# SamsungLabs/nb-asr

Measured on AMD Instinct MI355X. Metric: utterances_per_sec, higher is better.
Workload: dtype f32

## Files before the change

### nb_asr_amd/csrc/gemm_conv_split.hip

```cpp
#include "storage.h"

#include <cstdlib>

#include <type_traits>

namespace nbasr {

typedef float floatx4 __attribute__((ext_vector_type(4)));

constexpr int PB_CI = 16, PB_TAPS = 8;
constexpr int pb_frames(int nj) { return 64 * nj; }
constexpr int pb_rows(int mi) { return 32 * mi; }
constexpr int PB_THREADS = 512;

struct SplitBf16x3 {
    static constexpr int NS = 3;
    typedef __bf16 vec8 __attribute__((ext_vector_type(8)));
    static constexpr bool SCALED = false;
    __host__ __device__ static constexpr int taps_per_step(int stride) { return stride == 1 ? 4 : 2; }
    __device__ static __forceinline__ void split(float v, unsigned short (&s)[NS]) {
        const __bf16 hi = static_cast<__bf16>(v);
        const float r1 = v - static_cast<float>(hi);
        const __bf16 mid = static_cast<__bf16>(r1);
        const __bf16 lo = static_cast<__bf16>(r1 - static_cast<float>(mid));
        s[0] = __builtin_bit_cast(unsigned short, hi);
        s[1] = __builtin_bit_cast(unsigned short, mid);
        s[2] = __builtin_bit_cast(unsigned short, lo);
    }
    __device__ static __forceinline__ floatx4 mfma(vec8 a, vec8 b, floatx4 c) {
        return __builtin_amdgcn_mfma_f32_16x16x32_bf16(a, b, c, 0, 0, 0);
    }
    static constexpr const char* NAME = "nbasr_dense_conv1d_packed(bf16x3)";
};

struct SplitF16x2 {
    static constexpr int NS = 2;
    typedef _Float16 vec8 __attribute__((ext_vector_type(8)));
    static constexpr bool SCALED = true;
    __host__ __device__ static constexpr int taps_per_step(int) { return 4; }
    __device__ static __forceinline__ void split(float v, unsigned short (&s)[NS]) {
        const _Float16 hi = static_cast<_Float16>(v);
        const _Float16 lo = static_cast<_Float16>(v - static_cast<float>(hi));
        s[0] = __builtin_bit_cast(unsigned short, hi);
        s[1] = __builtin_bit_cast(unsigned short, lo);
    }
    __device__ static __forceinline__ floatx4 mfma(vec8 a, vec8 b, floatx4 c) {
        return __builtin_amdgcn_mfma_f32_16x16x32_f16(a, b, c, 0, 0, 0);
    }
    static constexpr const char* NAME = "nbasr_dense_conv1d_packed(f16x2)";
};

struct PlainBf16 {
    static constexpr int NS = 1;
    typedef __bf16 vec8 __attribute__((ext_vector_type(8)));
    static constexpr bool SCALED = false;
    __host__ __device__ static constexpr int taps_per_step(int) { return 8; }
    __device__ static __forceinline__ void split(float v, unsigned short (&s)[NS]) {
        s[0] = __builtin_bit_cast(unsigned short, static_cast<__bf16>(v));
    }
    __device__ static __forceinline__ floatx4 mfma(vec8 a, vec8 b, floatx4 c) {
        return __builtin_amdgcn_mfma_f32_16x16x32_bf16(a, b, c, 0, 0, 0);
    }
    static constexpr const char* NAME = "nbasr_dense_conv1d_packed(bf16)";
};

template <class P> constexpr bool has_image_path() { return P::SCALED || P::NS == 1; }

template <class P> constexpr size_t pb_group_bytes(int mi) { return static_cast<size_t>(P::NS) * PB_TAPS * pb_rows(mi) * PB_CI * 2; }

template <class P, int S, int MI = 4, int NJ = 4>
struct GeoP {
    static constexpr int PBM = pb_rows(MI);
    static constexpr int PBN = pb_frames(NJ);
    static constexpr int TP = P::taps_per_step(S);
    static constexpr int QSTEPS = PB_TAPS / TP;
    static constexpr int A_STEP_BYTES = P::NS * TP * PBM * PB_CI * 2;
    static constexpr int XR = (PBN - 1) * S + PB_TAPS;
    static constexpr int XRH = (XR + 1) / 2;
    static constexpr int ROWS = (S == 1) ? XR : 2 * XRH;
    static constexpr int RP = (ROWS + 15) / 16 * 16;
    static constexpr int X_BYTES = P::NS * RP * PB_CI * 2;
    static constexpr int NQUADS = ((XR + 3 + 3) / 4 + 7) / 8 * 8;
    static constexpr int XITEMS = NQUADS * (PB_CI / 2);
    static constexpr int NCHUNK = QSTEPS > 1 ? QSTEPS - 1 : 1;
    static constexpr int XI = (XITEMS + PB_THREADS * NCHUNK - 1) / (PB_THREADS * NCHUNK);
    static constexpr int RING = 2;
    static constexpr int OPERAND_BYTES = RING * (A_STEP_BYTES + X_BYTES);
    static constexpr int STAGING_BYTES = 8 * 32 * 68 * 4;
    static constexpr int LDS_BYTES = OPERAND_BYTES > STAGING_BYTES ? OPERAND_BYTES : STAGING_BYTES;
    __device__ static constexpr int rowmap(int row) { return (S == 1) ? row : (row & 1) * XRH + (row >> 1); }
};

struct PackedConvArgs {
    const float* x; const unsigned char* wp; const float* bias;
    const float* s0; const float* s1; const float* s2;
    float* y;
    int c_in, frames_in, ld_in, c_out, frames_out, ld_out, lpad;
    int n_groups, n_mt, n_nt, batch;
    LnRef ln_x;
    const float* x_absmax;
    const float* w_inv_scale;
    int x_is_image;
    const float* x_range;
    int sel_want;
    int staged_epilogue;
    float* part;
};

__device__ __forceinline__ bool range_is_extreme(const float* r) { return r[2] != 0.f || r[1] < r[0] * 2.44140625e-04f; }

__host__ __device__ inline void pow2_normaliser(float absmax, int target, float& scale, float& inv)
{
    unsigned bits;
    __builtin_memcpy(&bits, &absmax, 4);
    const int e = static_cast<int>((bits >> 23) & 0xffu);
    int k = (bits & 0x7fffffffu) ? (127 + target) - e : 0;
    k = k > 126 ? 126 : (k < -126 ? -126 : k);
    const unsigned sb = static_cast<unsigned>(127 + k) << 23, ib = static_cast<unsigned>(127 - k) << 23;
    __builtin_memcpy(&scale, &sb, 4);
    __builtin_memcpy(&inv, &ib, 4);
}

__device__ __forceinline__ unsigned pack2(unsigned short a, unsigned short b) {
    return static_cast<unsigned>(a) | (static_cast<unsigned>(b) << 16);
}

__global__ __launch_bounds__(256) void weight_row_scales_kernel(const float* __restrict__ w, float* __restrict__ scales,
                                                                int c_out, int row_elems, int rows)
{
    __shared__ float s_max[4];
    const int co = blockIdx.x;
    float m = 0.f;
    if (co < c_out)
        for (int i = threadIdx.x; i < row_elems; i += 256) m = fmaxf(m, fabsf(w[static_cast<size_t>(co) * row_elems + i]));
#pragma unroll
    for (int d = 32; d >= 1; d >>= 1) m = fmaxf(m, __shfl_xor(m, d));
    if ((threadIdx.x & 63) == 0) s_max[threadIdx.x >> 6] = m;
    __syncthreads();
    if (threadIdx.x == 0) {
        float scale, inv;
        pow2_normaliser(fmaxf(fmaxf(s_max[0], s_max[1]), fmaxf(s_max[2], s_max[3])), 13, scale, inv);
        scales[co] = scale;
        scales[rows + co] = inv;
    }
}

template <class P>
__global__ __launch_bounds__(256) void pack_dense_weights_kernel(const float* __restrict__ w, unsigned short* __restrict__ wp,
                                                                 const float* __restrict__ row_scale,
                                                                 int c_out, int c_in, int n_mt, int n_groups, int PB_TP, int PB_M)
{
    const int PB_QSTEPS = PB_TAPS / PB_TP;
    const long long total = static_cast<long long>(n_mt) * n_groups * PB_QSTEPS * PB_TP * PB_M * PB_CI;
    for (long long i = static_cast<long long>(blockIdx.x) * blockDim.x + threadIdx.x; i < total;
         i += static_cast<long long>(gridDim.x) * blockDim.x) {
        long long e = i;
        const int ci_l = e % PB_CI; e /= PB_CI;
        const int co_l = e % PB_M; e /= PB_M;
        const int tp = e % PB_TP; e /= PB_TP;
        const int q = e % PB_QSTEPS; e /= PB_QSTEPS;
        const int g = e % n_groups; e /= n_groups;
        const int mt = static_cast<int>(e);
        const int co = mt * PB_M + co_l, ci = g * PB_CI + ci_l, tap = q * PB_TP + tp;
        float v = (co < c_out && ci < c_in) ? w[(static_cast<size_t>(co) * c_in + ci) * PB_TAPS + tap] : 0.f;
        if (P::SCALED) v *= row_scale[co];
        unsigned short s[P::NS];
        P::split(v, s);
        const size_t step = (static_cast<size_t>(mt) * n_groups + g) * PB_QSTEPS + q;
#pragma unroll
        for (int k = 0; k < P::NS; ++k)
            wp[((((step * P::NS + k) * PB_TP + tp) * 2 + (ci_l >> 3)) * PB_M + co_l) * 8 + (ci_l & 7)] = s[k];
    }
}

template <class P, int S, bool LNX, bool XIMG = false, int MI = 4, int NJ = 4>
__global__ __launch_bounds__(PB_THREADS, 2) void gemm_conv_split_kernel(const PackedConvArgs a)
{
    static_assert(NJ == 4 || (NJ == 2 && XIMG && P::NS == 2) || (NJ == 8 && XIMG && P::NS == 1),
                  "128-frame tiles exist for the fp16 image path only, 512-frame tiles for the one-term bf16 flavour only");
    static_assert(!(XIMG && LNX) && !(XIMG && !has_image_path<P>()), "the image path: scaled fp16 scheme or plain bf16, no LayerNorm on load");
    static_assert(XIMG || P::NS > 1, "plain bf16 operands exist as an image only");
    static_assert(MI == 4 || ((MI == 5 || MI == 3 || MI == 2) && XIMG), "160-, 96- and 64-row tiles exist for the image path only");
    using G = GeoP<P, S, MI, NJ>;
    constexpr int PB_M = G::PBM, WROWS = 16 * MI;
    constexpr int PB_N = G::PBN, WCOLS = 16 * NJ;
    using vec8 = typename P::vec8;
    constexpr int TP = G::TP, QS = G::QSTEPS, ASTEP = G::A_STEP_BYTES;
    extern __shared__ __attribute__((aligned(16))) unsigned char smem[];
    unsigned char* const Abuf = smem;
    unsigned char* const Xbase = smem + G::RING * ASTEP;

    const int nwg = gridDim.x, id = blockIdx.x;
    const int xq = nwg >> 3, xr = nwg & 7, xcd = id & 7;
    const int L = (xcd < xr ? xcd * (xq + 1) : xr * (xq + 1) + (xcd - xr) * xq) + (id >> 3);
    int mt_i, b, nt_i;
    {
        mt_i = L % a.n_mt;
        const int rest = L / a.n_mt;
        b = rest / a.n_nt;
        nt_i = rest - b * a.n_nt;
    }
    const int m0 = mt_i * PB_M, n0 = nt_i * PB_N;
    if (a.x_range && a.sel_want >= 0 && static_cast<int>(range_is_extreme(a.x_range + 4 * b)) != a.sel_want) return;

    const int tid = threadIdx.x;
    const int lane = tid & 63;
    const int wave = __builtin_amdgcn_readfirstlane(tid >> 6);
    const int wm = wave >> 2, wn = wave & 3;
    const bool older = wave < 4;

    const float* __restrict__ xb = a.x + static_cast<size_t>(b) * a.c_in * a.ld_in;
    const int tin0 = n0 * S - a.lpad;
    const float* __restrict__ xstats = LNX ? a.ln_x.stats + static_cast<size_t>(b) * 2 * a.ld_in : nullptr;
    const unsigned char* __restrict__ wtile = a.wp + static_cast<size_t>(mt_i) * a.n_groups * pb_group_bytes<P>(MI);

    const bool wave_active = (m0 + wm * WROWS) < a.c_out && (n0 + wn * WCOLS) < a.ld_out;

    floatx4 acc[MI][NJ], tot[MI][NJ];
#pragma unroll
    for (int i = 0; i < MI; ++i)
#pragma unroll
        for (int j = 0; j < NJ; ++j)
#pragma unroll
            for (int r = 0; r < 4; ++r) { acc[i][j][r] = 0.f; tot[i][j][r] = 0.f; }
    auto flush_group = [&]() {
        if constexpr (P::NS > 1) {
#pragma unroll
            for (int i = 0; i < MI; ++i)
#pragma unroll
                for (int j = 0; j < NJ; ++j)
#pragma unroll
                    for (int r = 0; r < 4; ++r) { tot[i][j][r] += acc[i][j][r]; acc[i][j][r] = 0.f; }
        }
    };

    auto dma_weights = [&](int step, int buf) {
        const unsigned char* src = wtile + static_cast<size_t>(step) * ASTEP;
#pragma unroll
        for (int j = 0; j < ASTEP / 1024 / 8; ++j) {
            const int chunk = wave * (ASTEP / 1024 / 8) + j;
            __builtin_amdgcn_global_load_lds(
                (const __attribute__((address_space(1))) void*)(src + chunk * 1024 + lane * 16),
                (__attribute__((address_space(3))) void*)(Abuf + buf * ASTEP + chunk * 1024),
                16, 0, 0);
        }
    };
    auto dma_x = [&](int g, int xbuf, int q) {
        constexpr int NP = (G::X_BYTES + 1023) / 1024;
        const unsigned char* img = reinterpret_cast<const unsigned char*>(a.x) +
                                   (static_cast<size_t>(b) * a.n_groups + g) * (2 * P::NS) * static_cast<size_t>(a.ld_in + 1) * 16;
#pragma unroll 1
        for (int i = wave * QS + q; i < NP; i += 8 * QS) {
            const int o = i * 1024 + lane * 16;
            if (o < G::X_BYTES) {
                const int plane = o / (G::RP * 16), rr = (o - plane * (G::RP * 16)) >> 4;
                const int frame = tin0 + (S == 1 ? rr : 2 * (rr % G::XRH) + rr / G::XRH);
                const int row = (rr < G::ROWS && frame >= 0 && frame < a.ld_in) ? frame + 1 : 0;
                __builtin_amdgcn_global_load_lds(
                    (const __attribute__((address_space(1))) void*)(img + (static_cast<size_t>(plane) * (a.ld_in + 1) + row) * 16),
                    (__attribute__((address_space(3))) void*)(Xbase + xbuf * G::X_BYTES + i * 1024), 16, 0, 0);
            }
        }
    };
    floatx4 xreg[G::XI][2];
    const int a0 = tin0 & ~3, xoff = tin0 - a0;
    float x_scale = 1.f, x_inv = 1.f;
    if constexpr (P::SCALED) pow2_normaliser(a.x_range ? a.x_range[4 * b] : a.x_absmax[b], 14, x_scale, x_inv);
    auto load_x = [&](int g, int c) {
#pragma unroll
        for (int i = 0; i < G::XI; ++i) {
            const int e = tid + PB_THREADS * (c * G::XI + i);
            const int p = (e >> 3) & 7;
            const int t = a0 + 4 * ((e >> 6) * 8 + (e & 7));
            const int ci = g * PB_CI + 2 * p;
            const bool ok = e < G::XITEMS && t >= 0 && t < a.ld_in;
            floatx4 v0 = {0.f, 0.f, 0.f, 0.f}, v1 = {0.f, 0.f, 0.f, 0.f};
            if (ok && ci < a.c_in) v0 = *reinterpret_cast<const floatx4*>(xb + static_cast<size_t>(ci) * a.ld_in + t);
            if (ok && ci + 1 < a.c_in) v1 = *reinterpret_cast<const floatx4*>(xb + static_cast<size_t>(ci + 1) * a.ld_in + t);
            if (LNX && ok) {
                const floatx4 mean = *reinterpret_cast<const floatx4*>(xstats + t);
                const floatx4 rstd = *reinterpret_cast<const floatx4*>(xstats + a.ld_in + t);
                if (ci < a.c_in) {
                    const float gm = a.ln_x.gamma[ci], bt = a.ln_x.beta[ci];
#pragma unroll
                    for (int j = 0; j < 4; ++j) v0[j] = ln_apply(v0[j], mean[j], rstd[j], gm, bt);
                }
                if (ci + 1 < a.c_in) {
                    const float gm = a.ln_x.gamma[ci + 1], bt = a.ln_x.beta[ci + 1];
#pragma unroll
                    for (int j = 0; j < 4; ++j) v1[j] = ln_apply(v1[j], mean[j], rstd[j], gm, bt);
                }
            }
            if constexpr (P::SCALED) { v0 *= x_scale; v1 *= x_scale; }
            xreg[i][0] = v0;
            xreg[i][1] = v1;
        }
    };
    auto commit_x = [&](int xbuf, int c) {
        unsigned* const X = reinterpret_cast<unsigned*>(Xbase + xbuf * G::X_BYTES);
#pragma unroll
        for (int i = 0; i < G::XI; ++i) {
            const int e = tid + PB_THREADS * (c * G::XI + i);
            const int p = (e >> 3) & 7;
            const int row0 = 4 * ((e >> 6) * 8 + (e & 7)) - xoff;
            if (e >= G::XITEMS) continue;
            unsigned* const col = X + (p >> 2) * G::RP * 4 + (p & 3);
#pragma unroll
            for (int j = 0; j < 4; ++j) {
                const int row = row0 + j;
                if (row < 0 || row >= G::XR) continue;
                unsigned short s0[P::NS], s1[P::NS];
                P::split(xreg[i][0][j], s0);
                P::split(xreg[i][1][j], s1);
                unsigned* dst = col + G::rowmap(row) * 4;
#pragma unroll
                for (int k = 0; k < P::NS; ++k) dst[k * 2 * G::RP * 4] = pack2(s0[k], s1[k]);
            }
        }
    };

    const int l15 = lane & 15, kq = lane >> 4;
    const int a_lane = (((kq >> 1) * 2 + (kq & 1)) * PB_M + wm * WROWS + l15) * 16;
    const int x_lane = (kq & 1) * G::RP * 16;

    constexpr bool PIPE = P::NS <= 2;
    auto mma_step = [&](int q, int abuf, int xbuf) {
        const unsigned char* A = Abuf + abuf * ASTEP + a_lane;
        const unsigned char* X = Xbase + xbuf * G::X_BYTES + x_lane;
        auto read_b = [&](int pp, int j, vec8 (&f)[P::NS]) {
            const int row = G::rowmap((wn * WCOLS + j * 16 + l15) * S + q * TP + 2 * pp + (kq >> 1));
#pragma unroll
            for (int k = 0; k < P::NS; ++k) f[k] = *reinterpret_cast<const vec8*>(X + (k * 2 * G::RP + row) * 16);
        };
        auto read_a = [&](int pp, int i, vec8 (&f)[P::NS]) {
#pragma unroll
            for (int k = 0; k < P::NS; ++k) f[k] = *reinterpret_cast<const vec8*>(A + ((k * TP + 2 * pp) * 2 * PB_M + i * 16) * 16);
        };
        auto block = [&](int i, int j, const vec8 (&af)[P::NS], const vec8 (&bf)[P::NS]) {
            floatx4 c = acc[i][j];
            if constexpr (P::NS == 3) {
                c = P::mfma(af[2], bf[0], c);
                c = P::mfma(af[0], bf[2], c);
                c = P::mfma(af[1], bf[1], c);
            }
            if constexpr (P::NS > 1) {
                c = P::mfma(af[1], bf[0], c);
                c = P::mfma(af[0], bf[1], c);
            }
            acc[i][j] = P::mfma(af[0], bf[0], c);
        };
        if constexpr (PIPE) {
            vec8 bfr[NJ][P::NS], af[2][P::NS];
#pragma unroll
            for (int j = 0; j < NJ; ++j) read_b(0, j, bfr[j]);
            read_a(0, 0, af[0]);
#pragma unroll
            for (int pp = 0; pp < TP / 2; ++pp) {
#pragma unroll
                for (int i = 0; i < MI; ++i) {
                    const int cur = (pp * MI + i) & 1;
                    const bool more_a = i < MI - 1 || pp + 1 < TP / 2;
#pragma unroll
                    for (int j = 0; j < NJ; ++j) {
                        __builtin_amdgcn_sched_barrier(0);
                        block(i, j, af[cur], bfr[j]);
                        __builtin_amdgcn_sched_barrier(0);
                        if (j == 0 && more_a) read_a(i < MI - 1 ? pp : pp + 1, (i + 1) % MI, af[cur ^ 1]);
                        if (i == MI - 1 && pp + 1 < TP / 2) read_b(pp + 1, j, bfr[j]);
                    }
                }
            }
            __builtin_amdgcn_sched_barrier(0);
        } else {
#pragma unroll 1
            for (int pp = 0; pp < TP / 2; ++pp) {
                vec8 bfr[NJ][P::NS];
#pragma unroll
                for (int j = 0; j < NJ; ++j) read_b(pp, j, bfr[j]);
#pragma unroll
                for (int i = 0; i < MI; ++i) {
                    vec8 af[P::NS];
                    read_a(pp, i, af);
#pragma unroll
                    for (int j = 0; j < NJ; ++j) block(i, j, af, bfr[j]);
                }
            }
        }
    };

    const int ng = a.n_groups;
    dma_weights(0, 0);
    if constexpr (XIMG) {
#pragma unroll 1
        for (int q = 0; q < QS; ++q) dma_x(0, 0, q);
    } else {
#pragma unroll 1
        for (int c = 0; c < G::NCHUNK; ++c) { load_x(0, c); commit_x(0, c); }
    }
    asm volatile("s_waitcnt vmcnt(0)" ::: "memory");
    __syncthreads();

    if (!older) __builtin_amdgcn_s_setprio(1);
    int step = 0;
    for (int g = 0; g < ng; ++g) {
        const bool more = g + 1 < ng;
#pragma unroll 1
        for (int q = 0; q < QS; ++q, ++step) {
            const bool prefetch = q + 1 < QS || more;
            const bool chunk = more && q < QS - 1;
            if (older) {
                if constexpr (XIMG) {
                    if (more) dma_x(g + 1, (g + 1) & 1, q);
                } else {
                    if (more && q >= 1) commit_x((g + 1) & 1, q - 1);
                    if (chunk) load_x(g + 1, q);
                }
                if (prefetch) dma_weights(step + 1, (step + 1) & 1);
            } else if (!XIMG && chunk) {
                load_x(g + 1, q);
            }
            if (wave_active) mma_step(q, step & 1, g & 1);
            if (!older) {
                if constexpr (XIMG) {
                    if (more) dma_x(g + 1, (g + 1) & 1, q);
                } else {
                    if (chunk) commit_x((g + 1) & 1, q);
                }
                if (prefetch) dma_weights(step + 1, (step + 1) & 1);
            }
            asm volatile("s_waitcnt vmcnt(0)" ::: "memory");
            __syncthreads();
        }
        flush_group();
    }

    if constexpr (P::NS == 1) {
        constexpr int TSH = WCOLS + 8;
        constexpr int LPR = WCOLS / 8, RPI = 64 / LPR;
        unsigned short* const T = reinterpret_cast<unsigned short*>(smem) + wave * (32 * TSH);
        static_assert(8 * 32 * TSH * 2 <= G::LDS_BYTES, "output staging must fit the operand buffers");
        if (wave_active) {
            bf16_t* const yb = reinterpret_cast<bf16_t*>(a.y);
            const int n = n0 + wn * WCOLS + (lane % LPR) * 8;
#pragma unroll
            for (int i0 = 0; i0 < MI; i0 += 2) {
#pragma unroll
                for (int ii = 0; ii < 2; ++ii) {
                    const int i = i0 + ii;
                    if (i >= MI) break;
#pragma unroll
                    for (int j = 0; j < NJ; ++j) {
                        const bool live = n0 + wn * WCOLS + j * 16 + l15 < a.frames_out;
#pragma unroll
                        for (int r = 0; r < 4; ++r) {
                            const int m = m0 + wm * WROWS + i * 16 + kq * 4 + r;
                            const float v = (live && m < a.c_out) ? relu_clamp(acc[i][j][r] + a.bias[m]) : 0.f;
                            T[(ii * 16 + kq * 4 + r) * TSH + j * 16 + l15] = __builtin_bit_cast(unsigned short, static_cast<__bf16>(v));
                        }
                    }
                }
                asm volatile("s_waitcnt lgkmcnt(0)" ::: "memory");
                const int rows_pass = (MI - i0 >= 2) ? 32 : 16;
#pragma unroll
                for (int it = 0; it < 32 / RPI; ++it) {
                    const int ml = it * RPI + lane / LPR, m = m0 + wm * WROWS + i0 * 16 + ml;
                    if (ml < rows_pass && m < a.c_out && n < a.ld_out) {
                        const u4v t = *reinterpret_cast<const u4v*>(T + ml * TSH + (lane % LPR) * 8);
                        *reinterpret_cast<u4v*>(yb + (static_cast<size_t>(b) * a.c_out + m) * a.ld_out + n) = t;
                    }
                }
                asm volatile("s_waitcnt lgkmcnt(0)" ::: "memory");
            }
        }
        return;
    } else {
    if (!a.s0 && !a.s1 && !a.s2 && a.staged_epilogue) {
        constexpr int TS = WCOLS + 4;
        constexpr int FQ = WCOLS / 4, RI = 64 / FQ, NIT = 32 / RI;
        float* const T = reinterpret_cast<float*>(smem) + wave * (32 * TS);
        static_assert(8 * 32 * TS * 4 <= G::LDS_BYTES, "output staging must fit the operand buffers");
        if (!wave_active) return;
        const int nc = n0 + wn * WCOLS + (lane % FQ) * 4;
        const bool want_stats = a.part != nullptr;
        const int scol = lane % WCOLS, usel = lane / WCOLS;
        const int ncol = n0 + wn * WCOLS + scol;
#pragma unroll
        for (int i0 = 0; i0 < MI; i0 += 2) {
#pragma unroll
            for (int ii = 0; ii < 2; ++ii) {
                const int i = i0 + ii;
                if (i >= MI) break;
#pragma unroll
                for (int j = 0; j < NJ; ++j) {
                    const bool live = n0 + wn * WCOLS + j * 16 + l15 < a.frames_out;
#pragma unroll
                    for (int r = 0; r < 4; ++r) {
                        const int m = m0 + wm * WROWS + i * 16 + kq * 4 + r;
                        float v = 0.f;
                        if (live && m < a.c_out) {
                            float sum = tot[i][j][r];
                            if constexpr (P::SCALED) sum = sum * x_inv * a.w_inv_scale[m];
                            v = relu_clamp(sum + a.bias[m]);
                        }
                        T[(ii * 16 + kq * 4 + r) * TS + j * 16 + l15] = v;
                    }
                }
            }
            asm volatile("s_waitcnt lgkmcnt(0)" ::: "memory");
            const int rows_pass = (MI - i0 >= 2) ? 32 : 16;
#pragma unroll
            for (int it = 0; it < NIT; ++it) {
                const int ml = it * RI + lane / FQ;
                const int m = m0 + wm * WROWS + i0 * 16 + ml;
                if (ml < rows_pass && m < a.c_out && nc < a.ld_out) {
                    const floatx4 t = *reinterpret_cast<const floatx4*>(T + ml * TS + (lane % FQ) * 4);
                    *reinterpret_cast<floatx4*>(a.y + (static_cast<size_t>(b) * a.c_out + m) * a.ld_out + nc) = t;
                }
            }
            if (want_stats) {
#pragma unroll
                for (int u0 = 0; u0 < 2; u0 += 64 / WCOLS) {
                    const int u = u0 + usel;
                    const int mu = m0 + wm * WROWS + (i0 + u) * 16;
                    if (i0 + u < MI && mu < a.c_out) {
                        const int nrows = min(16, a.c_out - mu);
                        const float c = T[(u * 16) * TS + scol];
                        float s1 = 0.f, s2 = 0.f;
#pragma unroll
                        for (int r = 1; r < 16; ++r) {
                            const float d = (r < nrows) ? T[(u * 16 + r) * TS + scol] - c : 0.f;
                            s1 += d;
                            s2 = __builtin_fmaf(d, d, s2);
                        }
                        if (ncol < a.ld_out) {
                            const float inv = 1.0f / static_cast<float>(nrows);
                            float* prow = a.part + (static_cast<size_t>(mu >> 4) * a.batch + b) * 2 * a.ld_out + ncol;
                            prow[0] = c + s1 * inv;
                            prow[a.ld_out] = s2 - s1 * s1 * inv;
                        }
                    }
                }
            }
            asm volatile("s_waitcnt lgkmcnt(0)" ::: "memory");
        }
        return;
    }
    if (!wave_active) return;
#pragma unroll
    for (int i = 0; i < MI; ++i) {
#pragma unroll
        for (int j = 0; j < NJ; ++j) {
            const int n = n0 + wn * WCOLS + j * 16 + l15;
            if (n >= a.ld_out) continue;
            const bool live = n < a.frames_out;
#pragma unroll
            for (int r = 0; r < 4; ++r) {
                const int m = m0 + wm * WROWS + i * 16 + kq * 4 + r;
                if (m >= a.c_out) continue;
                float sum = tot[i][j][r];
                if constexpr (P::SCALED) sum = sum * x_inv * a.w_inv_scale[m];
                float v = relu_clamp(sum + a.bias[m]);
                const size_t off = (static_cast<size_t>(b) * a.c_out + m) * a.ld_out + n;
                if (a.s0) v += a.s0[off];
                if (a.s1) v += a.s1[off];
                if (a.s2) v += a.s2[off];
                a.y[off] = live ? v : 0.f;
            }
        }
    }
    }
}


template <class P, int S>
static int launch_packed(PackedConvArgs a, hipStream_t stream)
{
    using G = GeoP<P, S>;
    constexpr int PB_M = G::PBM;
    constexpr bool HAS_LNX = !P::SCALED;
    static const hipError_t attr0 = hipFuncSetAttribute(reinterpret_cast<const void*>(gemm_conv_split_kernel<P, S, false>),
                                                        hipFuncAttributeMaxDynamicSharedMemorySize, G::LDS_BYTES);
    static const hipError_t attr1 = hipFuncSetAttribute(reinterpret_cast<const void*>(gemm_conv_split_kernel<P, S, HAS_LNX>),
                                                        hipFuncAttributeMaxDynamicSharedMemorySize, G::LDS_BYTES);
    const hipError_t attr = attr0 != hipSuccess ? attr0 : attr1;
    if (attr != hipSuccess) {
        set_error("%s: cannot reserve %d bytes of LDS: %s", P::NAME, G::LDS_BYTES, hipGetErrorString(attr));
        return static_cast<int>(attr);
    }
    NBASR_REQUIRE(HAS_LNX || !a.ln_x.stats, NBASR_EINVAL, "%s: this scheme takes no deferred LayerNorm", P::NAME);
    a.n_mt = (a.c_out + PB_M - 1) / PB_M;
    a.n_nt = (a.ld_out + G::PBN - 1) / G::PBN;
    const long long nwg = static_cast<long long>(a.n_mt) * a.n_nt * a.batch;
    NBASR_REQUIRE(nwg < (1ll << 31), NBASR_EINVAL, "%s: too many tiles (%lld)", P::NAME, nwg);
    if (a.ln_x.stats)
        hipLaunchKernelGGL((gemm_conv_split_kernel<P, S, HAS_LNX>), dim3(static_cast<unsigned>(nwg)), dim3(PB_THREADS), G::LDS_BYTES, stream, a);
    else
        hipLaunchKernelGGL((gemm_conv_split_kernel<P, S, false>), dim3(static_cast<unsigned>(nwg)), dim3(PB_THREADS), G::LDS_BYTES, stream, a);
    return launch_status(P::NAME);
}

static inline int rows_to_mi(int row_tile) { return row_tile == 128 ? 4 : (row_tile == 160 ? 5 : (row_tile == 96 ? 3 : (row_tile == 64 ? 2 : 0))); }

template <class P, int S, int MI, int NJ = 4>
static int launch_image(PackedConvArgs a, hipStream_t stream)
{
    using G = GeoP<P, S, MI, NJ>;
    static const hipError_t attr = hipFuncSetAttribute(reinterpret_cast<const void*>(gemm_conv_split_kernel<P, S, false, true, MI, NJ>),
                                                       hipFuncAttributeMaxDynamicSharedMemorySize, G::LDS_BYTES);
    if (attr != hipSuccess) {
        set_error("%s: cannot reserve %d bytes of LDS: %s", P::NAME, G::LDS_BYTES, hipGetErrorString(attr));
        return static_cast<int>(attr);
    }
    a.n_mt = (a.c_out + G::PBM - 1) / G::PBM;
    a.n_nt = (a.ld_out + G::PBN - 1) / G::PBN;
    const long long nwg = static_cast<long long>(a.n_mt) * a.n_nt * a.batch;
    NBASR_REQUIRE(nwg < (1ll << 31), NBASR_EINVAL, "%s: too many tiles (%lld)", P::NAME, nwg);
    hipLaunchKernelGGL((gemm_conv_split_kernel<P, S, false, true, MI, NJ>), dim3(static_cast<unsigned>(nwg)), dim3(PB_THREADS), G::LDS_BYTES, stream, a);
    return launch_status(P::NAME);
}

template <class P>
static size_t packed_bytes(int c_out, int c_in, int kernel, int row_tile = 128)
{
    const int mi = rows_to_mi(row_tile);
    if (c_out <= 0 || c_in <= 0 || kernel != PB_TAPS || mi == 0 || (mi != 4 && !has_image_path<P>())) return 0;
    const size_t PB_M = pb_rows(mi), n_mt = (c_out + PB_M - 1) / PB_M, n_groups = (c_in + PB_CI - 1) / PB_CI;
    return n_mt * n_groups * pb_group_bytes<P>(mi) + (P::SCALED ? 2 * n_mt * PB_M * sizeof(float) : 0);
}

template <class P>
static int pack_impl(const float* w, void* packed, int c_out, int c_in, int kernel, int stride, nbasr_stream_t stream, int row_tile = 128)
{
    clear_error();
    const int mi = rows_to_mi(row_tile);
    NBASR_REQUIRE(mi != 0 && (mi == 4 || has_image_path<P>()), NBASR_EINVAL, "nbasr_pack_dense_weights: row_tile=%d unsupported (128, or 64 / 96 / 160 for the image-path schemes)", row_tile);
    const int PB_M = pb_rows(mi);
    NBASR_REQUIRE(c_out > 0 && c_in > 0, NBASR_EINVAL, "nbasr_pack_dense_weights: bad sizes");
    NBASR_REQUIRE(kernel == PB_TAPS && (stride == 1 || stride == 2), NBASR_EINVAL,
                  "nbasr_pack_dense_weights: (kernel=%d, stride=%d) unsupported (the downsample convs have k=8, s in {1,2})", kernel, stride);
    NBASR_REQUIRE(w && packed, NBASR_ENULL, "nbasr_pack_dense_weights: NULL pointer");
    NBASR_REQUIRE(aligned16(packed), NBASR_EALIGN, "nbasr_pack_dense_weights: packed buffer must be 16-byte aligned");
    const int n_mt = (c_out + PB_M - 1) / PB_M, n_groups = (c_in + PB_CI - 1) / PB_CI;
    float* scales = nullptr;
    if (P::SCALED) {
        scales = reinterpret_cast<float*>(static_cast<unsigned char*>(packed) + static_cast<size_t>(n_mt) * n_groups * pb_group_bytes<P>(mi));
        hipLaunchKernelGGL(weight_row_scales_kernel, dim3(n_mt * PB_M), dim3(256), 0, as_stream(stream), w, scales, c_out,
                           c_in * PB_TAPS, n_mt * PB_M);
    }
    hipLaunchKernelGGL(pack_dense_weights_kernel<P>, dim3(2048), dim3(256), 0, as_stream(stream), w,
                       static_cast<unsigned short*>(packed), scales, c_out, c_in, n_mt, n_groups, P::taps_per_step(stride), PB_M);
    return launch_status("nbasr_pack_dense_weights");
}

template <class P>
static int dense_packed_impl(const float* x, const void* packed_w, const float* bias, const float* skip0,
                             const float* skip1, const float* skip2, float* y, int batch, int c_in,
                             int frames_in, int ld_in, int c_out, int ld_out, int kernel, int stride,
                             const nbasr_deferred_ln* ln, const float* x_absmax, nbasr_stream_t stream, bool x_is_image = false,
                             int row_tile = 128, const float* x_range = nullptr, int sel_want = -1, float* stats_part = nullptr,
                             int frame_tile = 256)
{
    clear_error();
    const int mi = rows_to_mi(row_tile);
    NBASR_REQUIRE(mi == 4 || ((mi == 5 || mi == 3 || mi == 2) && x_is_image && P::SCALED), NBASR_EINVAL,
                  "%s: row_tile=%d unsupported (128; 64, 96 and 160 for the fp16 image path)", P::NAME, row_tile);
    const int PB_M = pb_rows(mi);
    NBASR_REQUIRE(frame_tile == 256 || (frame_tile == 128 && x_is_image && P::SCALED), NBASR_EINVAL,
                  "%s: frame_tile=%d unsupported (256; 128 for the fp16 image path)", P::NAME, frame_tile);
    NBASR_REQUIRE(batch >= 0 && c_in > 0 && c_out > 0 && frames_in >= 0, NBASR_EINVAL, "%s: bad sizes", P::NAME);
    NBASR_REQUIRE(kernel == PB_TAPS && (stride == 1 || stride == 2), NBASR_EINVAL,
                  "%s: (kernel=%d, stride=%d) unsupported; packed path covers k=8, s in {1,2}", P::NAME, kernel, stride);
    const int frames_out = (frames_in + stride - 1) / stride;
    NBASR_REQUIRE(ld_in >= frames_in, NBASR_EINVAL, "%s: ld_in=%d < frames_in=%d", P::NAME, ld_in, frames_in);
    NBASR_REQUIRE(ld_in % 4 == 0, NBASR_EALIGN, "%s: ld_in=%d must be a multiple of 4", P::NAME, ld_in);
    NBASR_REQUIRE(ld_out >= frames_out && ld_out % 4 == 0, NBASR_EALIGN,
                  "%s: ld_out=%d must be >= %d output frames and a multiple of 4", P::NAME, ld_out, frames_out);
    if (batch == 0 || frames_out == 0) return NBASR_OK;
    NBASR_REQUIRE(x && packed_w && bias && y, NBASR_ENULL, "%s: x, packed_w, bias, y must be non-NULL", P::NAME);
    NBASR_REQUIRE(aligned16(packed_w) && aligned16(x), NBASR_EALIGN, "%s: x and packed weights must be 16-byte aligned", P::NAME);
    PackedConvArgs a{};
    a.x = x; a.wp = static_cast<const unsigned char*>(packed_w); a.bias = bias; a.s0 = skip0; a.s1 = skip1; a.s2 = skip2; a.y = y;
    a.c_in = c_in; a.frames_in = frames_in; a.ld_in = ld_in; a.c_out = c_out; a.frames_out = frames_out; a.ld_out = ld_out;
    a.lpad = pad_left(kernel, 1, stride); a.n_groups = (c_in + PB_CI - 1) / PB_CI; a.batch = batch;
    NBASR_REQUIRE(!ln || (ln->stats && ln->gamma && ln->beta), NBASR_ENULL, "%s: deferred LayerNorm needs stats, gamma and beta", P::NAME);
    a.ln_x = ln_ref(ln, true);
    a.x_range = x_range;
    a.sel_want = x_range ? sel_want : -1;
    a.staged_epilogue = 1;
    NBASR_REQUIRE(!stats_part || (!skip0 && !skip1 && !skip2 && aligned16(stats_part)), NBASR_EINVAL,
                  "%s: the statistics by-product exists for the skip-free convolution only (stats_part 16-byte aligned)", P::NAME);
    a.part = stats_part;
    if (P::SCALED) {
        NBASR_REQUIRE(x_absmax || x_range, NBASR_ENULL, "%s: x_absmax (per-utterance bound of |x|) must be non-NULL", P::NAME);
        a.x_absmax = x_absmax;
        a.x_is_image = x_is_image ? 1 : 0;
        a.w_inv_scale = reinterpret_cast<const float*>(a.wp + static_cast<size_t>((c_out + PB_M - 1) / PB_M) * a.n_groups * pb_group_bytes<P>(mi))
                        + static_cast<size_t>((c_out + PB_M - 1) / PB_M) * PB_M;
    }
    if constexpr (has_image_path<P>() && P::SCALED) {
        if (x_is_image) {
// ... 120 lines not shown
```

Before: 11040.

## Make image-path conv GEMM persistent with next-tile prefetch during epilogue

Converts the image-path conv GEMM into a persistent kernel whose grid is capped at the resident workgroup count, with each workgroup looping over tiles. When the LDS budget allows, the first step's weights, activations and the bias and scale rows for the next tile are DMA'd into LDS while the current tile's epilogue runs. Kernel args are read through the kernarg pointer. The intent is to hide launch tail and per-tile prologue latency. The cost is extra LDS per workgroup, which can reduce occupancy, plus more complex synchronisation.

Measured after the change: 11040, median of 2. About the same (+0.0%).

```diff
diff --git a/nb_asr_amd/csrc/gemm_conv_split.hip b/nb_asr_amd/csrc/gemm_conv_split.hip
--- a/nb_asr_amd/csrc/gemm_conv_split.hip
+++ b/nb_asr_amd/csrc/gemm_conv_split.hip
@@ -3,6 +3,10 @@
 #include <cstdlib>
 
 #include <type_traits>
+
+#ifndef NBASR_DENSE_STAMPS
+#define NBASR_DENSE_STAMPS 0
+#endif
 
 namespace nbasr {
 
@@ -88,6 +92,13 @@
     static constexpr int OPERAND_BYTES = RING * (A_STEP_BYTES + X_BYTES);
     static constexpr int STAGING_BYTES = 8 * 32 * 68 * 4;
     static constexpr int LDS_BYTES = OPERAND_BYTES > STAGING_BYTES ? OPERAND_BYTES : STAGING_BYTES;
+    static constexpr int SLOT_BYTES = A_STEP_BYTES + X_BYTES;
+    static constexpr bool FETCH_AHEAD = LDS_BYTES > 80 * 1024;
+    static constexpr int OUT_BYTES = P::NS == 1 ? 8 * 32 * (16 * NJ + 8) * 2 : 8 * 32 * (16 * NJ + 4) * 4;
+    static constexpr int ROWVEC_BYTES = 2 * PBM * 4;
+    static constexpr int ROWVEC_OFFSET = OPERAND_BYTES > SLOT_BYTES + OUT_BYTES ? OPERAND_BYTES : SLOT_BYTES + OUT_BYTES;
+    static constexpr int IMAGE_LDS_BYTES = FETCH_AHEAD ? ROWVEC_OFFSET + 2 * ROWVEC_BYTES : LDS_BYTES;
+    static_assert(IMAGE_LDS_BYTES <= 160 * 1024, "one workgroup must fit the compute unit's LDS");
     __device__ static constexpr int rowmap(int row) { return (S == 1) ? row : (row & 1) * XRH + (row >> 1); }
 };
 
@@ -105,6 +116,9 @@
     int sel_want;
     int staged_epilogue;
     float* part;
+#if NBASR_DENSE_STAMPS
+    unsigned long long* stamps;
+#endif
 };
 
 __device__ __forceinline__ bool range_is_extreme(const float* r) { return r[2] != 0.f || r[1] < r[0] * 2.44140625e-04f; }
@@ -174,8 +188,11 @@
 }
 
 template <class P, int S, bool LNX, bool XIMG = false, int MI = 4, int NJ = 4>
-__global__ __launch_bounds__(PB_THREADS, 2) void gemm_conv_split_kernel(const PackedConvArgs a)
-{
+__global__ __launch_bounds__(PB_THREADS, 2) void gemm_conv_split_kernel(const PackedConvArgs args)
+{
+    typedef const __attribute__((address_space(4))) PackedConvArgs* ArgsPtr;
+    ArgsPtr a = (ArgsPtr)__builtin_amdgcn_kernarg_segment_ptr();
+    (void)args;
     static_assert(NJ == 4 || (NJ == 2 && XIMG && P::NS == 2) || (NJ == 8 && XIMG && P::NS == 1),
                   "128-frame tiles exist for the fp16 image path only, 512-frame tiles for the one-term bf16 flavour only");
     static_assert(!(XIMG && LNX) && !(XIMG && !has_image_path<P>()), "the image path: scaled fp16 scheme or plain bf16, no LayerNorm on load");
@@ -187,21 +204,58 @@
     using vec8 = typename P::vec8;
     constexpr int TP = G::TP, QS = G::QSTEPS, ASTEP = G::A_STEP_BYTES;
     extern __shared__ __attribute__((aligned(16))) unsigned char smem[];
+    constexpr int A_PITCH = XIMG ? G::SLOT_BYTES : ASTEP, X_PITCH = XIMG ? G::SLOT_BYTES : G::X_BYTES;
+    constexpr bool AHEAD = XIMG && G::FETCH_AHEAD;
     unsigned char* const Abuf = smem;
-    unsigned char* const Xbase = smem + G::RING * ASTEP;
-
-    const int nwg = gridDim.x, id = blockIdx.x;
-    const int xq = nwg >> 3, xr = nwg & 7, xcd = id & 7;
-    const int L = (xcd < xr ? xcd * (xq + 1) : xr * (xq + 1) + (xcd - xr) * xq) + (id >> 3);
+    unsigned char* const Xbase = smem + (XIMG ? ASTEP : G::RING * ASTEP);
+    unsigned char* const stage = smem + (AHEAD ? G::SLOT_BYTES : 0);
+    float* const rowvec = reinterpret_cast<float*>(smem + (AHEAD ? G::ROWVEC_OFFSET : 0));
+
+    const int ntiles = a->n_mt * a->n_nt * a->batch;
+    auto decode = [&](int id, int& mt, int& bb, int& nt) {
+        const int xq = ntiles >> 3, xr = ntiles & 7, xcd = id & 7;
+        const int L = (xcd < xr ? xcd * (xq + 1) : xr * (xq + 1) + (xcd - xr) * xq) + (id >> 3);
+        mt = L % a->n_mt;
+        const int rest = L / a->n_mt;
+        bb = rest / a->n_nt;
+        nt = rest - bb * a->n_nt;
+    };
+    auto next_tile = [&](int id) {
+        if (a->x_range && a->sel_want >= 0) {
+            for (; id < ntiles; id += static_cast<int>(gridDim.x)) {
+                int mt, bb, nt;
+                decode(id, mt, bb, nt);
+                if (static_cast<int>(range_is_extreme(a->x_range + 4 * bb)) == a->sel_want) break;
+            }
+        }
+        return id < ntiles ? id : ntiles;
+    };
+    int tile = next_tile(blockIdx.x);
+    if (tile >= ntiles) return;
     int mt_i, b, nt_i;
-    {
-        mt_i = L % a.n_mt;
-        const int rest = L / a.n_mt;
-        b = rest / a.n_nt;
-        nt_i = rest - b * a.n_nt;
-    }
-    const int m0 = mt_i * PB_M, n0 = nt_i * PB_N;
-    if (a.x_range && a.sel_want >= 0 && static_cast<int>(range_is_extreme(a.x_range + 4 * b)) != a.sel_want) return;
+    decode(tile, mt_i, b, nt_i);
+    int m0 = mt_i * PB_M, n0 = nt_i * PB_N;
+#if NBASR_DENSE_STAMPS
+    unsigned long long* stamp_row = nullptr;
+    int stamp_i = 2;
+    auto stamp = [&]() {
+        if (stamp_row && threadIdx.x == 0) stamp_row[stamp_i] = wall_clock64();
+        ++stamp_i;
+    };
+    auto stamp_tile = [&]() {
+        stamp_row = (XIMG && a->stamps) ? a->stamps + static_cast<size_t>(tile) * 8 : nullptr;
+        stamp_i = 2;
+        if (stamp_row && threadIdx.x == 0) {
+            stamp_row[0] = __builtin_amdgcn_s_getreg(4 | (31 << 11));
+            stamp_row[1] = __builtin_amdgcn_s_getreg(20 | (31 << 11));
+        }
+        stamp();
+    };
+#else
+    auto stamp = []() {};
+    auto stamp_tile = []() {};
+#endif
+    stamp_tile();
 
     const int tid = threadIdx.x;
     const int lane = tid & 63;
@@ -209,20 +263,14 @@
     const int wm = wave >> 2, wn = wave & 3;
     const bool older = wave < 4;
 
-    const float* __restrict__ xb = a.x + static_cast<size_t>(b) * a.c_in * a.ld_in;
-    const int tin0 = n0 * S - a.lpad;
-    const float* __restrict__ xstats = LNX ? a.ln_x.stats + static_cast<size_t>(b) * 2 * a.ld_in : nullptr;
-    const unsigned char* __restrict__ wtile = a.wp + static_cast<size_t>(mt_i) * a.n_groups * pb_group_bytes<P>(MI);
-
-    const bool wave_active = (m0 + wm * WROWS) < a.c_out && (n0 + wn * WCOLS) < a.ld_out;
+    const float* __restrict__ xb = a->x + static_cast<size_t>(b) * a->c_in * a->ld_in;
+    int tin0 = n0 * S - a->lpad;
+    const float* __restrict__ xstats = LNX ? a->ln_x.stats + static_cast<size_t>(b) * 2 * a->ld_in : nullptr;
+    const unsigned char* __restrict__ wtile = a->wp + static_cast<size_t>(mt_i) * a->n_groups * pb_group_bytes<P>(MI);
+
+    bool wave_active = (m0 + wm * WROWS) < a->c_out && (n0 + wn * WCOLS) < a->ld_out;
 
     floatx4 acc[MI][NJ], tot[MI][NJ];
-#pragma unroll
-    for (int i = 0; i < MI; ++i)
-#pragma unroll
-        for (int j = 0; j < NJ; ++j)
-#pragma unroll
-            for (int r = 0; r < 4; ++r) { acc[i][j][r] = 0.f; tot[i][j][r] = 0.f; }
     auto flush_group = [&]() {
         if constexpr (P::NS > 1) {
 #pragma unroll
@@ -234,38 +282,64 @@
         }
     };
 
-    auto dma_weights = [&](int step, int buf) {
-        const unsigned char* src = wtile + static_cast<size_t>(step) * ASTEP;
+    auto dma_weights_of = [&](const unsigned char* wt, int step, int buf, int wave, int lane) {
+        const unsigned char* src = wt + static_cast<size_t>(step) * ASTEP;
 #pragma unroll
         for (int j = 0; j < ASTEP / 1024 / 8; ++j) {
             const int chunk = wave * (ASTEP / 1024 / 8) + j;
             __builtin_amdgcn_global_load_lds(
                 (const __attribute__((address_space(1))) void*)(src + chunk * 1024 + lane * 16),
-                (__attribute__((address_space(3))) void*)(Abuf + buf * ASTEP + chunk * 1024),
+                (__attribute__((address_space(3))) void*)(Abuf + buf * A_PITCH + chunk * 1024),
                 16, 0, 0);
         }
     };
-    auto dma_x = [&](int g, int xbuf, int q) {
+    auto dma_weights = [&](int step, int buf) { dma_weights_of(wtile, step, buf, wave, lane); };
+    auto dma_x_of = [&](int bb, int tin, int g, int xbuf, int q, int wave, int lane) {
         constexpr int NP = (G::X_BYTES + 1023) / 1024;
-        const unsigned char* img = reinterpret_cast<const unsigned char*>(a.x) +
-                                   (static_cast<size_t>(b) * a.n_groups + g) * (2 * P::NS) * static_cast<size_t>(a.ld_in + 1) * 16;
+        const unsigned char* img = reinterpret_cast<const unsigned char*>(a->x) +
+                                   (static_cast<size_t>(bb) * a->n_groups + g) * (2 * P::NS) * static_cast<size_t>(a->ld_in + 1) * 16;
 #pragma unroll 1
         for (int i = wave * QS + q; i < NP; i += 8 * QS) {
             const int o = i * 1024 + lane * 16;
             if (o < G::X_BYTES) {
                 const int plane = o / (G::RP * 16), rr = (o - plane * (G::RP * 16)) >> 4;
-                const int frame = tin0 + (S == 1 ? rr : 2 * (rr % G::XRH) + rr / G::XRH);
-                const int row = (rr < G::ROWS && frame >= 0 && frame < a.ld_in) ? frame + 1 : 0;
+                const int frame = tin + (S == 1 ? rr : 2 * (rr % G::XRH) + rr / G::XRH);
+                const int row = (rr < G::ROWS && frame >= 0 && frame < a->ld_in) ? frame + 1 : 0;
                 __builtin_amdgcn_global_load_lds(
-                    (const __attribute__((address_space(1))) void*)(img + (static_cast<size_t>(plane) * (a.ld_in + 1) + row) * 16),
-                    (__attribute__((address_space(3))) void*)(Xbase + xbuf * G::X_BYTES + i * 1024), 16, 0, 0);
-            }
-        }
+                    (const __attribute__((address_space(1))) void*)(img + (static_cast<size_t>(plane) * (a->ld_in + 1) + row) * 16),
+                    (__attribute__((address_space(3))) void*)(Xbase + xbuf * X_PITCH + i * 1024), 16, 0, 0);
+            }
+        }
+    };
+    auto dma_x = [&](int g, int xbuf, int q) { dma_x_of(b, tin0, g, xbuf, q, wave, lane); };
+    auto dma_rowvec = [&](int mt, int sel, int wave, int lane) {
+        if constexpr (AHEAD) {
+            const int part = wave & 3, rl = part * 64 + lane;
+            const bool second = wave >= 4;
+            if (part * 64 < PB_M && (P::SCALED || !second)) {
+                const float* src = second ? a->w_inv_scale : a->bias;
+                if (rl < PB_M && mt * PB_M + rl < a->c_out)
+                    __builtin_amdgcn_global_load_lds(
+                        (const __attribute__((address_space(1))) void*)(src + mt * PB_M + rl),
+                        (__attribute__((address_space(3))) void*)(rowvec + (sel * 2 + (second ? 1 : 0)) * PB_M + part * 64), 4, 0, 0);
+            }
+        }
+    };
+    auto fetch_step0 = [&](const unsigned char* wt, int mt, int bb, int tin, int sel) {
+        int wave_f = wave, lane_f = lane;
+        if constexpr (AHEAD) asm volatile("" : "+s"(wave_f), "+v"(lane_f));
+        dma_weights_of(wt, 0, 0, wave_f, lane_f);
+#pragma unroll 1
+        for (int q = 0; q < QS; ++q) dma_x_of(bb, tin, 0, 0, q, wave_f, lane_f);
+        dma_rowvec(mt, sel, wave_f, lane_f);
     };
     floatx4 xreg[G::XI][2];
     const int a0 = tin0 & ~3, xoff = tin0 - a0;
     float x_scale = 1.f, x_inv = 1.f;
-    if constexpr (P::SCALED) pow2_normaliser(a.x_range ? a.x_range[4 * b] : a.x_absmax[b], 14, x_scale, x_inv);
+    auto set_x_scale = [&](int bb) {
+        if constexpr (P::SCALED) pow2_normaliser(a->x_range ? a->x_range[4 * bb] : a->x_absmax[bb], 14, x_scale, x_inv);
+    };
+    set_x_scale(b);
     auto load_x = [&](int g, int c) {
 #pragma unroll
         for (int i = 0; i < G::XI; ++i) {
@@ -273,20 +347,20 @@
             const int p = (e >> 3) & 7;
             const int t = a0 + 4 * ((e >> 6) * 8 + (e & 7));
             const int ci = g * PB_CI + 2 * p;
-            const bool ok = e < G::XITEMS && t >= 0 && t < a.ld_in;
+            const bool ok = e < G::XITEMS && t >= 0 && t < a->ld_in;
             floatx4 v0 = {0.f, 0.f, 0.f, 0.f}, v1 = {0.f, 0.f, 0.f, 0.f};
-            if (ok && ci < a.c_in) v0 = *reinterpret_cast<const floatx4*>(xb + static_cast<size_t>(ci) * a.ld_in + t);
-            if (ok && ci + 1 < a.c_in) v1 = *reinterpret_cast<const floatx4*>(xb + static_cast<size_t>(ci + 1) * a.ld_in + t);
+            if (ok && ci < a->c_in) v0 = *reinterpret_cast<const floatx4*>(xb + static_cast<size_t>(ci) * a->ld_in + t);
+            if (ok && ci + 1 < a->c_in) v1 = *reinterpret_cast<const floatx4*>(xb + static_cast<size_t>(ci + 1) * a->ld_in + t);
             if (LNX && ok) {
                 const floatx4 mean = *reinterpret_cast<const floatx4*>(xstats + t);
-                const floatx4 rstd = *reinterpret_cast<const floatx4*>(xstats + a.ld_in + t);
-                if (ci < a.c_in) {
-                    const float gm = a.ln_x.gamma[ci], bt = a.ln_x.beta[ci];
+                const floatx4 rstd = *reinterpret_cast<const floatx4*>(xstats + a->ld_in + t);
+                if (ci < a->c_in) {
+                    const float gm = a->ln_x.gamma[ci], bt = a->ln_x.beta[ci];
 #pragma unroll
                     for (int j = 0; j < 4; ++j) v0[j] = ln_apply(v0[j], mean[j], rstd[j], gm, bt);
                 }
-                if (ci + 1 < a.c_in) {
-                    const float gm = a.ln_x.gamma[ci + 1], bt = a.ln_x.beta[ci + 1];
+                if (ci + 1 < a->c_in) {
+                    const float gm = a->ln_x.gamma[ci + 1], bt = a->ln_x.beta[ci + 1];
 #pragma unroll
                     for (int j = 0; j < 4; ++j) v1[j] = ln_apply(v1[j], mean[j], rstd[j], gm, bt);
                 }
@@ -325,8 +399,8 @@
 
     constexpr bool PIPE = P::NS <= 2;
     auto mma_step = [&](int q, int abuf, int xbuf) {
-        const unsigned char* A = Abuf + abuf * ASTEP + a_lane;
-        const unsigned char* X = Xbase + xbuf * G::X_BYTES + x_lane;
+        const unsigned char* A = Abuf + abuf * A_PITCH + a_lane;
+        const unsigned char* X = Xbase + xbuf * X_PITCH + x_lane;
         auto read_b = [&](int pp, int j, vec8 (&f)[P::NS]) {
             const int row = G::rowmap((wn * WCOLS + j * 16 + l15) * S + q * TP + 2 * pp + (kq >> 1));
 #pragma unroll
@@ -388,19 +462,30 @@
         }
     };
 
-    const int ng = a.n_groups;
-    dma_weights(0, 0);
+    const int ng = a->n_groups;
+    int sel = 0;
     if constexpr (XIMG) {
-#pragma unroll 1
-        for (int q = 0; q < QS; ++q) dma_x(0, 0, q);
+        fetch_step0(wtile, mt_i, b, tin0, sel);
     } else {
+        dma_weights(0, 0);
 #pragma unroll 1
         for (int c = 0; c < G::NCHUNK; ++c) { load_x(0, c); commit_x(0, c); }
     }
     asm volatile("s_waitcnt vmcnt(0)" ::: "memory");
-    __syncthreads();
 
     if (!older) __builtin_amdgcn_s_setprio(1);
+    for (;;) {
+    if constexpr (XIMG) asm volatile("" : "+s"(a));
+    if constexpr (AHEAD) asm volatile("s_waitcnt lgkmcnt(0)\n\ts_barrier" ::: "memory");
+    else __syncthreads();
+    stamp();
+    int nxt = XIMG ? next_tile(tile + static_cast<int>(gridDim.x)) : ntiles;
+#pragma unroll
+    for (int i = 0; i < MI; ++i)
+#pragma unroll
+        for (int j = 0; j < NJ; ++j)
+#pragma unroll
+            for (int r = 0; r < 4; ++r) { acc[i][j][r] = 0.f; tot[i][j][r] = 0.f; }
     int step = 0;
     for (int g = 0; g < ng; ++g) {
         const bool more = g + 1 < ng;
@@ -433,14 +518,44 @@
         }
         flush_group();
     }
-
+    stamp();
+
+    if constexpr (XIMG) asm volatile("" : "+s"(a), "+s"(nxt));
+    if constexpr (AHEAD) {
+        if (nxt < ntiles) {
+            int nmt, nb, nnt;
+            decode(nxt, nmt, nb, nnt);
+            fetch_step0(a->wp + static_cast<size_t>(nmt) * a->n_groups * pb_group_bytes<P>(MI), nmt, nb, nnt * PB_N * S - a->lpad, sel ^ 1);
+        }
+    }
+
+    auto epilogue = [&]() {
+    int lane_e = lane, wave_e = wave;
+    asm volatile("" : "+v"(lane_e), "+s"(wave_e));
+    const int lane = lane_e, wave = wave_e;
+    const int l15 = lane & 15, kq = lane >> 4, wm = wave >> 2, wn = wave & 3;
+    if constexpr (XIMG) asm volatile("" : "+s"(a));
+    struct EpilogueArgs {
+        const float* bias; const float* w_inv_scale; const float* s0; const float* s1; const float* s2; float* y; float* part;
+        int c_out, frames_out, ld_out, batch, staged_epilogue;
+    };
+    const EpilogueArgs args_e{a->bias, a->w_inv_scale, a->s0, a->s1, a->s2, a->y, a->part,
+                              a->c_out, a->frames_out, a->ld_out, a->batch, a->staged_epilogue};
+    const EpilogueArgs* const a = &args_e;
+    auto bias_of = [&](int m) { return AHEAD ? rowvec[(sel * 2) * PB_M + (m - m0)] : a->bias[m]; };
+    auto w_inv_of = [&](int m) { return AHEAD ? rowvec[(sel * 2 + 1) * PB_M + (m - m0)] : a->w_inv_scale[m]; };
+    auto ahead_landed = [&](bool last_pass) {
+        if constexpr (AHEAD) {
+            if (last_pass) asm volatile("s_waitcnt vmcnt(0)" ::: "memory");
+        }
+    };
     if constexpr (P::NS == 1) {
         constexpr int TSH = WCOLS + 8;
         constexpr int LPR = WCOLS / 8, RPI = 64 / LPR;
-        unsigned short* const T = reinterpret_cast<unsigned short*>(smem) + wave * (32 * TSH);
-        static_assert(8 * 32 * TSH * 2 <= G::LDS_BYTES, "output staging must fit the operand buffers");
+        unsigned short* const T = reinterpret_cast<unsigned short*>(stage) + wave * (32 * TSH);
+        static_assert(8 * 32 * TSH * 2 <= (AHEAD ? G::OUT_BYTES : G::LDS_BYTES), "output staging must fit the operand buffers");
         if (wave_active) {
-            bf16_t* const yb = reinterpret_cast<bf16_t*>(a.y);
+            bf16_t* const yb = reinterpret_cast<bf16_t*>(a->y);
             const int n = n0 + wn * WCOLS + (lane % LPR) * 8;
 #pragma unroll
             for (int i0 = 0; i0 < MI; i0 += 2) {
@@ -450,23 +565,24 @@
                     if (i >= MI) break;
 #pragma unroll
                     for (int j = 0; j < NJ; ++j) {
-                        const bool live = n0 + wn * WCOLS + j * 16 + l15 < a.frames_out;
+                        const bool live = n0 + wn * WCOLS + j * 16 + l15 < a->frames_out;
 #pragma unroll
                         for (int r = 0; r < 4; ++r) {
                             const int m = m0 + wm * WROWS + i * 16 + kq * 4 + r;
-                            const float v = (live && m < a.c_out) ? relu_clamp(acc[i][j][r] + a.bias[m]) : 0.f;
+                            const float v = (live && m < a->c_out) ? relu_clamp(acc[i][j][r] + bias_of(m)) : 0.f;
                             T[(ii * 16 + kq * 4 + r) * TSH + j * 16 + l15] = __builtin_bit_cast(unsigned short, static_cast<__bf16>(v));
                         }
                     }
                 }
                 asm volatile("s_waitcnt lgkmcnt(0)" ::: "memory");
                 const int rows_pass = (MI - i0 >= 2) ? 32 : 16;
+                ahead_landed(i0 + 2 >= MI);
 #pragma unroll
                 for (int it = 0; it < 32 / RPI; ++it) {
                     const int ml = it * RPI + lane / LPR, m = m0 + wm * WROWS + i0 * 16 + ml;
-                    if (ml < rows_pass && m < a.c_out && n < a.ld_out) {
+                    if (ml < rows_pass && m < a->c_out && n < a->ld_out) {
                         const u4v t = *reinterpret_cast<const u4v*>(T + ml * TSH + (lane % LPR) * 8);
-                        *reinterpret_cast<u4v*>(yb + (static_cast<size_t>(b) * a.c_out + m) * a.ld_out + n) = t;
+                        *reinterpret_cast<u4v*>(yb + (static_cast<size_t>(b) * a->c_out + m) * a->ld_out + n) = t;
                     }
                 }
                 asm volatile("s_waitcnt lgkmcnt(0)" ::: "memory");
@@ -474,14 +590,14 @@
         }
         return;
     } else {
-    if (!a.s0 && !a.s1 && !a.s2 && a.staged_epilogue) {
+    if (XIMG || (!a->s0 && !a->s1 && !a->s2 && a->staged_epilogue)) {
         constexpr int TS = WCOLS + 4;
         constexpr int FQ = WCOLS / 4, RI = 64 / FQ, NIT = 32 / RI;
-        float* const T = reinterpret_cast<float*>(smem) + wave * (32 * TS);
-        static_assert(8 * 32 * TS * 4 <= G::LDS_BYTES, "output staging must fit the operand buffers");
+        float* const T = reinterpret_cast<float*>(stage) + wave * (32 * TS);
+        static_assert(8 * 32 * TS * 4 <= (AHEAD ? G::OUT_BYTES : G::LDS_BYTES), "output staging must fit the operand buffers");
         if (!wave_active) return;
         const int nc = n0 + wn * WCOLS + (lane % FQ) * 4;
-        const bool want_stats = a.part != nullptr;
+        const bool want_stats = a->part != nullptr;
         const int scol = lane % WCOLS, usel = lane / WCOLS;
         const int ncol = n0 + wn * WCOLS + scol;
 #pragma unroll
@@ -492,15 +608,15 @@
                 if (i >= MI) break;
 #pragma unroll
                 for (int j = 0; j < NJ; ++j) {
-                    const bool live = n0 + wn * WCOLS + j * 16 + l15 < a.frames_out;
+                    const bool live = n0 + wn * WCOLS + j * 16 + l15 < a->frames_out;
 #pragma unroll
                     for (int r = 0; r < 4; ++r) {
                         const int m = m0 + wm * WROWS + i * 16 + kq * 4 + r;
                         float v = 0.f;
-                        if (live && m < a.c_out) {
+                        if (live && m < a->c_out) {
                             float sum = tot[i][j][r];
-                            if constexpr (P::SCALED) sum = sum * x_inv * a.w_inv_scale[m];
-                            v = relu_clamp(sum + a.bias[m]);
+                            if constexpr (P::SCALED) sum = sum * x_inv * w_inv_of(m);
+                            v = relu_clamp(sum + bias_of(m));
                         }
                         T[(ii * 16 + kq * 4 + r) * TS + j * 16 + l15] = v;
                     }
@@ -508,13 +624,14 @@
             }
             asm volatile("s_waitcnt lgkmcnt(0)" ::: "memory");
             const int rows_pass = (MI - i0 >= 2) ? 32 : 16;
+            ahead_landed(i0 + 2 >= MI);
 #pragma unroll
             for (int it = 0; it < NIT; ++it) {
                 const int ml = it * RI + lane / FQ;
                 const int m = m0 + wm * WROWS + i0 * 16 + ml;
-                if (ml < rows_pass && m < a.c_out && nc < a.ld_out) {
+                if (ml < rows_pass && m < a->c_out && nc < a->ld_out) {
                     const floatx4 t = *reinterpret_cast<const floatx4*>(T + ml * TS + (lane % FQ) * 4);
-                    *reinterpret_cast<floatx4*>(a.y + (static_cast<size_t>(b) * a.c_out + m) * a.ld_out + nc) = t;
+                    *reinterpret_cast<floatx4*>(a->y + (static_cast<size_t>(b) * a->c_out + m) * a->ld_out + nc) = t;
                 }
             }
             if (want_stats) {
@@ -522,8 +639,8 @@
                 for (int u0 = 0; u0 < 2; u0 += 64 / WCOLS) {
                     const int u = u0 + usel;
                     const int mu = m0 + wm * WROWS + (i0 + u) * 16;
-                    if (i0 + u < MI && mu < a.c_out) {
-                        const int nrows = min(16, a.c_out - mu);
+                    if (i0 + u < MI && mu < a->c_out) {
+                        const int nrows = min(16, a->c_out - mu);
                         const float c = T[(u * 16) * TS + scol];
                         float s1 = 0.f, s2 = 0.f;
 #pragma unroll
@@ -532,11 +649,11 @@
                             s1 += d;
                             s2 = __builtin_fmaf(d, d, s2);
                         }
-                        if (ncol < a.ld_out) {
+                        if (ncol < a->ld_out) {
                             const float inv = 1.0f / static_cast<float>(nrows);
-                            float* prow = a.part + (static_cast<size_t>(mu >> 4) * a.batch + b) * 2 * a.ld_out + ncol;
+                            float* prow = a->part + (static_cast<size_t>(mu >> 4) * a->batch + b) * 2 * a->ld_out + ncol;
                             prow[0] = c + s1 * inv;
-                            prow[a.ld_out] = s2 - s1 * s1 * inv;
+                            prow[a->ld_out] = s2 - s1 * s1 * inv;
                         }
                     }
                 }
@@ -545,30 +662,63 @@
         }
         return;
     }
+    if constexpr (!XIMG) {
     if (!wave_active) return;
 #pragma unroll
     for (int i = 0; i < MI; ++i) {
 #pragma unroll
         for (int j = 0; j < NJ; ++j) {
             const int n = n0 + wn * WCOLS + j * 16 + l15;
-            if (n >= a.ld_out) continue;
-            const bool live = n < a.frames_out;
+            if (n >= a->ld_out) continue;
+            const bool live = n < a->frames_out;
 #pragma unroll
             for (int r = 0; r < 4; ++r) {
                 const int m = m0 + wm * WROWS + i * 16 + kq * 4 + r;
-                if (m >= a.c_out) continue;
+                if (m >= a->c_out) continue;
                 float sum = tot[i][j][r];
-                if constexpr (P::SCALED) sum = sum * x_inv * a.w_inv_scale[m];
-                float v = relu_clamp(sum + a.bias[m]);
-                const size_t off = (static_cast<size_t>(b) * a.c_out + m) * a.ld_out + n;
-                if (a.s0) v += a.s0[off];
-                if (a.s1) v += a.s1[off];
-                if (a.s2) v += a.s2[off];
-                a.y[off] = live ? v : 0.f;
-            }
-        }
-    }
-    }
+                if constexpr (P::SCALED) sum = sum * x_inv * a->w_inv_scale[m];
+                float v = relu_clamp(sum + a->bias[m]);
+                const size_t off = (static_cast<size_t>(b) * a->c_out + m) * a->ld_out + n;
+                if (a->s0) v += a->s0[off];
+                if (a->s1) v += a->s1[off];
+                if (a->s2) v += a->s2[off];
+                a->y[off] = live ? v : 0.f;
+            }
+        }
+    }
+    }
+    }
+    };
+    epilogue();
+    stamp();
+    if constexpr (XIMG) asm volatile("" : "+s"(nxt));
+    if (nxt >= ntiles) break;
+    if constexpr (AHEAD) {
+        if (!wave_active) asm volatile("s_waitcnt vmcnt(0)" ::: "memory");
+    }
+    stamp();
+
+    tile = nxt;
+    decode(tile, mt_i, b, nt_i);
+    m0 = mt_i * PB_M; n0 = nt_i * PB_N;
+    tin0 = n0 * S - a->lpad;
+    wtile = a->wp + static_cast<size_t>(mt_i) * a->n_groups * pb_group_bytes<P>(MI);
+    {
+        int wave_t = wave;
+        asm volatile("" : "+s"(wave_t));
+        wave_active = (m0 + (wave_t >> 2) * WROWS) < a->c_out && (n0 + (wave_t & 3) * WCOLS) < a->ld_out;
+    }
+    set_x_scale(b);
+    stamp_tile();
+    if constexpr (AHEAD) {
+        sel ^= 1;
+    } else {
+        __syncthreads();
+        fetch_step0(wtile, mt_i, b, tin0, 0);
+        asm volatile("s_waitcnt vmcnt(0)" ::: "memory");
+    }
+    }
+    stamp();
 }
 
 
@@ -605,17 +755,32 @@
 static int launch_image(PackedConvArgs a, hipStream_t stream)
 {
     using G = GeoP<P, S, MI, NJ>;
-    static const hipError_t attr = hipFuncSetAttribute(reinterpret_cast<const void*>(gemm_conv_split_kernel<P, S, false, true, MI, NJ>),
-                                                       hipFuncAttributeMaxDynamicSharedMemorySize, G::LDS_BYTES);
+    const void* const kernel = reinterpret_cast<const void*>(gemm_conv_split_kernel<P, S, false, true, MI, NJ>);
+    static const hipError_t attr = hipFuncSetAttribute(kernel, hipFuncAttributeMaxDynamicSharedMemorySize, G::IMAGE_LDS_BYTES);
     if (attr != hipSuccess) {
-        set_error("%s: cannot reserve %d bytes of LDS: %s", P::NAME, G::LDS_BYTES, hipGetErrorString(attr));
+        set_error("%s: cannot reserve %d bytes of LDS: %s", P::NAME, G::IMAGE_LDS_BYTES, hipGetErrorString(attr));
         return static_cast<int>(attr);
     }
+    static const long long resident = [kernel]() -> long long {
+        int per_cu = 0, dev = 0, cus = 0;
+        if (hipOccupancyMaxActiveBlocksPerMultiprocessor(&per_cu, kernel, PB_THREADS, G::IMAGE_LDS_BYTES) != hipSuccess || per_cu < 1) return 0;
+        if (hipGetDevice(&dev) != hipSuccess || hipDeviceGetAttribute(&cus, hipDeviceAttributeMultiprocessorCount, dev) != hipSuccess) return 0;
+        return static_cast<long long>(per_cu) * cus;
+    }();
+    NBASR_REQUIRE(resident > 0, NBASR_EINVAL, "%s: no workgroup of this instance fits a compute unit (%d bytes of LDS)", P::NAME, G::IMAGE_LDS_BYTES);
     a.n_mt = (a.c_out + G::PBM - 1) / G::PBM;
     a.n_nt = (a.ld_out + G::PBN - 1) / G::PBN;
-    const long long nwg = static_cast<long long>(a.n_mt) * a.n_nt * a.batch;
-    NBASR_REQUIRE(nwg < (1ll << 31), NBASR_EINVAL, "%s: too many tiles (%lld)", P::NAME, nwg);
-    hipLaunchKernelGGL((gemm_conv_split_kernel<P, S, false, true, MI, NJ>), dim3(static_cast<unsigned>(nwg)), dim3(PB_THREADS), G::LDS_BYTES, stream, a);
+    const long long tiles = static_cast<long long>(a.n_mt) * a.n_nt * a.batch;
+    NBASR_REQUIRE(tiles < (1ll << 30), NBASR_EINVAL, "%s: too many tiles (%lld)", P::NAME, tiles);
+    long long nwg = tiles < resident ? tiles : resident;
+    if (const char* e = getenv("NBASR_DENSE_GRID_CAP")) {
+        const long long cap = strtoll(e, nullptr, 10);
+        if (cap >= 1 && cap < nwg) nwg = cap;
+    }
+#if NBASR_DENSE_STAMPS
+    { const char* e = getenv("NBASR_DENSE_STAMPS"); a.stamps = e ? reinterpret_cast<unsigned long long*>(strtoull(e, nullptr, 0)) : nullptr; }
+#endif
+    hipLaunchKernelGGL((gemm_conv_split_kernel<P, S, false, true, MI, NJ>), dim3(static_cast<unsigned>(nwg)), dim3(PB_THREADS), G::IMAGE_LDS_BYTES, stream, a);
     return launch_status(P::NAME);
 }
 
```
